# cc-ai/climategan

Measured on AMD Instinct MI355X. Metric: 640x640 images/sec (G+D step): per-domain sample slots per second of the joint Masker+Painter training step (update_G + update_D), global batch 32 per domain, higher is better.
Workload: dtype bf16

## Files before the change

### climategan_amd/csrc/conv1x1_xres.hip

```cpp
#include "conv_gemm.h"
#include <type_traits>

namespace {

typedef float f32x2 __attribute__((ext_vector_type(2)));

__device__ __attribute__((aligned(16))) unsigned int g_xres_zeros[4];

__device__ __forceinline__ float row16_sum_x(float v) {
  v += __builtin_bit_cast(float, __builtin_amdgcn_update_dpp(0, __builtin_bit_cast(int, v), 0x128, 0xf, 0xf, false));
  v += __builtin_bit_cast(float, __builtin_amdgcn_update_dpp(0, __builtin_bit_cast(int, v), 0x124, 0xf, 0xf, false));
  v += __builtin_bit_cast(float, __builtin_amdgcn_update_dpp(0, __builtin_bit_cast(int, v), 0x122, 0xf, 0xf, false));
  v += __builtin_bit_cast(float, __builtin_amdgcn_update_dpp(0, __builtin_bit_cast(int, v), 0x121, 0xf, 0xf, false));
  return v;
}

template <int I, int N, typename F>
__device__ __forceinline__ void static_for(F&& f) {
  if constexpr (I < N) {
    f(std::integral_constant<int, I>{});
    static_for<I + 1, N>(f);
  }
}

template <typename T, int KC, int PF>
__global__ __launch_bounds__(512, 1) void conv1x1_xres_kernel(ConvGemmArgs p, int npb, unsigned long long* ts) {
  constexpr int WC = 4, WP = 8;
  constexpr int NKS = 2 * KC;
  constexpr int XCHUNK = 32 * 1024;
  constexpr int ROWB = WC * 32 + 16;
  constexpr int STG = 16 * ROWB;
  static_assert(NKS % PF == 0, "the prefetch ring must divide the k-steps (static register indices)");
  static_assert(KC * XCHUNK + 8 * STG <= 160 * 1024, "LDS");
  extern __shared__ __attribute__((aligned(1024))) unsigned char smem[];

  const int lane = threadIdx.x & 63;
  const int wave = __builtin_amdgcn_readfirstlane(threadIdx.x >> 6);
  const int xcd = blockIdx.x & 7, slot = blockIdx.x >> 3;
  const int pblk = xcd * ((npb + 7) >> 3) + slot;
  if (pblk >= npb) return;
  auto stamp = [&](int i) {
    if (ts && lane == 0 && i < 16) ts[((size_t)blockIdx.x * 8 + wave) * 16 + i] = __builtin_readcyclecounter();
  };
  stamp(0);

  {
    const long zero_off = reinterpret_cast<const unsigned char*>(g_xres_zeros) - reinterpret_cast<const unsigned char*>(p.x);
    const int q = lane >> 3;
#pragma unroll
    for (int m = 0; m < KC * 4; ++m) {
      const int id = wave + 8 * m;
      const int cc2 = id >> 5, t = (id & 31) >> 1, half = id & 1;
      const int kchunk = (lane & 7) ^ (4 * half + ((q >> 1) & 3));
      const int pix = (pblk * 16 + t) * 16 + 8 * half + q;
      const long off = pix < p.npix ? ((long)pix * p.cin_s + cc2 * 64 + kchunk * 8) * 2 : zero_off;
      __builtin_amdgcn_global_load_lds(
          (const __attribute__((address_space(1))) void*)(reinterpret_cast<const unsigned char*>(p.x) + off),
          (__attribute__((address_space(3))) void*)(smem + id * 1024), 16, 0, 0);
    }
  }

  const int wc = wave & 3, wp = wave >> 2;
  const int j16 = lane & 15, g = lane >> 4;
  const int ncb = (p.ctiles + 15) >> 4;
  int b_off[2];
  {
    const int q = j16 & 7, h = j16 >> 3;
#pragma unroll
    for (int c = 0; c < 2; ++c) b_off[c] = wp * WP * 2048 + 1024 * h + 128 * q + 16 * ((4 * c + g) ^ (4 * h + ((q >> 1) & 3)));
  }
  const __amdgpu_buffer_rsrc_t rs_w =
      __builtin_amdgcn_make_buffer_rsrc(const_cast<u32x4*>(p.w), 0, p.ctiles * p.ksteps * 1024, 0x00020000);
  const __amdgpu_buffer_rsrc_t rs_y = __builtin_amdgcn_make_buffer_rsrc(p.y, 0, p.npix * p.cout_s * 2, 0x00020000);
  const int lane16 = lane * 16;
  u32x4 a[PF][WC];
  auto load_a = [&](auto slot_tag, int cb, int ks) {
    constexpr int sl = decltype(slot_tag)::value;
#pragma unroll
    for (int c = 0; c < WC; ++c) {
      const int ct = min(cb * 16 + wc * WC + c, p.ctiles - 1);
      a[sl][c] = __builtin_amdgcn_raw_buffer_load_b128(rs_w, lane16, (ct * p.ksteps + ks) * 1024, 0);
    }
  };
  static_for<0, PF>([&](auto i) { load_a(i, 0, decltype(i)::value); });

  asm volatile("s_waitcnt vmcnt(0)" ::: "memory");
  __builtin_amdgcn_s_barrier();
  stamp(1);

  unsigned char* stg = smem + KC * XCHUNK + wave * STG;
  const int st_rd = (lane >> 3) * ROWB + (lane & 7) * 16;
  const int st_voff = ((lane >> 3) * p.cout_s + (lane & 7) * 8) * 2;
  const int pix_wave = (pblk * 16 + wp * WP) * 16;

  u32x4 b_lo[4], b_hi[4];
  auto read_b = [&](u32x4* bh, int ks, int half) {
#pragma unroll
    for (int t = 0; t < 4; ++t)
      bh[t] = *reinterpret_cast<const u32x4*>(smem + (ks >> 1) * XCHUNK + b_off[ks & 1] + (half * 4 + t) * 2048);
  };

  for (int cb = 0; cb < ncb; ++cb) {
    read_b(b_lo, 0, 0);
    f32x4 acc[WC][WP];
#pragma unroll
    for (int c = 0; c < WC; ++c)
#pragma unroll
      for (int t = 0; t < WP; ++t) acc[c][t] = (f32x4){0.f, 0.f, 0.f, 0.f};

    auto kstep = [&](auto ks_tag) {
      constexpr int ks = decltype(ks_tag)::value;
      constexpr int sl = ks % PF;
      read_b(b_hi, ks, 1);
      __builtin_amdgcn_sched_barrier(0);
#pragma unroll
      for (int t = 0; t < 4; ++t)
#pragma unroll
        for (int c = 0; c < WC; ++c) acc[c][t] = mfma16(as_vec8<T>(a[sl][c]), as_vec8<T>(b_lo[t]), acc[c][t]);
      __builtin_amdgcn_sched_barrier(0);
      if constexpr (ks + 1 < NKS) read_b(b_lo, ks + 1, 0);
      __builtin_amdgcn_sched_barrier(0);
#pragma unroll
      for (int t = 0; t < 4; ++t)
#pragma unroll
        for (int c = 0; c < WC; ++c) acc[c][4 + t] = mfma16(as_vec8<T>(a[sl][c]), as_vec8<T>(b_hi[t]), acc[c][4 + t]);
      __builtin_amdgcn_sched_barrier(0);
      if constexpr (ks + PF < NKS) load_a(std::integral_constant<int, sl>{}, cb, ks + PF);
      __builtin_amdgcn_sched_barrier(0);
    };
    static_for<0, NKS>(kstep);
    stamp(2 + 2 * cb);

    const int cout_base = (cb * 16 + wc * WC) * 16;
    const bool full = pix_wave + WP * 16 <= p.npix && cout_base + WC * 16 <= p.cout_s;
    if (p.stats && pix_wave < p.npix) {
      const int chunk = pblk * 2 + wp;
      constexpr float inv_cnt = 1.f / (float)(WP * 16);
#pragma unroll
      for (int c = 0; c < WC; ++c) {
        f32x2 vr[WP][2];
#pragma unroll
        for (int t = 0; t < WP; ++t) {
#pragma unroll
          for (int hh = 0; hh < 2; ++hh) {
            float r0, r1;
            unpack2<T>(pack2<T>(acc[c][t][2 * hh], acc[c][t][2 * hh + 1]), r0, r1);
            vr[t][hh] = (f32x2){r0, r1};
          }
        }
        f32x2 s0[2] = {vr[0][0], vr[0][1]};
#pragma unroll
        for (int t = 1; t < WP; ++t) {
          s0[0] += vr[t][0];
          s0[1] += vr[t][1];
        }
        float mean[4];
#pragma unroll
        for (int r = 0; r < 4; ++r) mean[r] = row16_sum_x(s0[r >> 1][r & 1]) * inv_cnt;
        const f32x2 m2[2] = {(f32x2){mean[0], mean[1]}, (f32x2){mean[2], mean[3]}};
        f32x2 s1[2];
#pragma unroll
        for (int hh = 0; hh < 2; ++hh) {
          const f32x2 dv = vr[0][hh] - m2[hh];
          s1[hh] = dv * dv;
        }
#pragma unroll
        for (int t = 1; t < WP; ++t)
#pragma unroll
          for (int hh = 0; hh < 2; ++hh) {
            const f32x2 dv = vr[t][hh] - m2[hh];
            s1[hh] += dv * dv;
          }
        float o[8];
#pragma unroll
        for (int r = 0; r < 4; ++r) {
          o[2 * r] = mean[r];
          o[2 * r + 1] = row16_sum_x(s1[r >> 1][r & 1]);
        }
        const int ch = cout_base + c * 16 + 4 * g;
        if (j16 == 0 && ch < p.cout_s) {
          float* dst = p.stats + ((size_t)chunk * p.cout_s + ch) * 2;
          *reinterpret_cast<f32x4*>(dst) = (f32x4){o[0], o[1], o[2], o[3]};
          *reinterpret_cast<f32x4*>(dst + 4) = (f32x4){o[4], o[5], o[6], o[7]};
        }
      }
    }
    auto emit = [&](auto full_tag) {
      constexpr bool FULL = decltype(full_tag)::value;
#pragma unroll
      for (int t = 0; t < WP; ++t) {
#pragma unroll
        for (int c = 0; c < WC; ++c) {
          const f32x4 v = acc[c][t];
          *reinterpret_cast<u32x2*>(stg + j16 * ROWB + c * 32 + g * 8) = (u32x2){pack2<T>(v[0], v[1]), pack2<T>(v[2], v[3])};
        }
        asm volatile("s_waitcnt lgkmcnt(0)" ::: "memory");
#pragma unroll
        for (int it = 0; it < 2; ++it) {
          const u32x4 o = *reinterpret_cast<const u32x4*>(stg + st_rd + it * 8 * ROWB);
          const int pix0 = pix_wave + t * 16 + it * 8;
          if (FULL || (pix0 + (lane >> 3) < p.npix && cout_base + (lane & 7) * 8 < p.cout_s))
            __builtin_amdgcn_raw_buffer_store_b128(o, rs_y, st_voff, (pix0 * p.cout_s + cout_base) * 2, 2);
        }
        asm volatile("s_waitcnt lgkmcnt(0)" ::: "memory");
        if (t == WP / 2 - 1 && cb + 1 < ncb) {
          __builtin_amdgcn_sched_barrier(0);
          static_for<0, PF>([&](auto i) { load_a(i, cb + 1, decltype(i)::value); });
          __builtin_amdgcn_sched_barrier(0);
        }
      }
    };
    if (full) emit(std::true_type{});
    else emit(std::false_type{});
    stamp(3 + 2 * cb);
  }
}

CGAN_KNOB(unsigned long long*, g_xres_ts, nullptr);

template <typename T, int KC, int PF>
int launch_xres(const ConvGemmArgs& a, hipStream_t s) {
  constexpr size_t smem = (size_t)KC * 32 * 1024 + 8 * 16 * (4 * 32 + 16);
  static bool attr_set = false;
  if (!attr_set) {
    hipError_t e = hipFuncSetAttribute(reinterpret_cast<const void*>(&conv1x1_xres_kernel<T, KC, PF>),
                                       hipFuncAttributeMaxDynamicSharedMemorySize, 160 * 1024);
    if (e != hipSuccess) {
      cgan_set_error("conv1x1_xres: hipFuncSetAttribute failed: %s", hipGetErrorString(e));
      return CGAN_ERR_HIP;
    }
    attr_set = true;
  }
  const int npb = ceil_div(a.npix, 256);
  hipLaunchKernelGGL((conv1x1_xres_kernel<T, KC, PF>), dim3(ceil_div(npb, 8) * 8), dim3(512), smem, s, a, npb, g_xres_ts);
  return CGAN_OK;
}

template <typename T>
int launch_any(const ConvGemmArgs& a, hipStream_t s) {
  switch (a.cin_s >> 6) {
    case 1: return launch_xres<T, 1, 2>(a, s);
    case 2: return launch_xres<T, 2, 2>(a, s);
    case 3: return launch_xres<T, 3, 2>(a, s);
    default: return launch_xres<T, 4, 2>(a, s);
  }
}

}

CGAN_DEV_ONLY(extern "C" void cgan_debug_set_xres_tsbuf(void* p) { g_xres_ts = (unsigned long long*)p; })

bool conv1x1_xres_ok(const ConvGemmArgs& a) {
  return a.kh == 1 && a.kw == 1 && a.stride == 1 && a.pad == 0 && (a.cin_s & 63) == 0 && a.cin_s <= 256 && !a.has_res &&
         !a.bias && a.act == CGAN_ACT_NONE && a.cout == a.cout_s &&
         a.h_in == a.h_out && a.w_in == a.w_out && (long)a.npix * a.cin_s < (1L << 30) &&
         (long)a.npix * a.cout_s < (1L << 30);
}

int conv1x1_xres_launch(const ConvGemmArgs& a, int dtype, hipStream_t s) {
  return dtype == CGAN_F16 ? launch_any<F16>(a, s) : launch_any<BF16>(a, s);
}
```

### climategan_amd/csrc/conv_gemm.h

```cpp
#pragma once
#include "cgan_common.h"

struct ConvGemmArgs {
  const uint16_t* x;
  const u32x4* w;
  const float* bias;
  const uint16_t* res;
  const uint16_t* res2;
  uint16_t* y;
  int n, h_in, w_in, cin_s;
  int cout, cout_s, ctiles, ksteps;
  int kh, kw, stride, pad, dil, pad_mode;
  int h_out, w_out, npix;
  int act, has_res, res_ups;
  float slope;
  float* stats;
};

struct ConvGemmCls {
  int koff;
  int kh, kw;
  int offy, offx;
};
struct ConvGemmExtArgs {
  ConvGemmArgs a;
  int cls_s;
  int ksplit;
  int ks_per;
  float* ws;
  int pair;
  ConvGemmCls cls[4];
};
bool conv_gemm_ext_shape_ok(const ConvGemmArgs& a);
int conv_gemm_splitk_plan(const ConvGemmArgs& a);
size_t conv_gemm_splitk_workspace_bytes(const ConvGemmArgs& a, int ksplit);
int conv_gemm_splitk_launch(const ConvGemmArgs& a, int ksplit, float* ws, int dtype, hipStream_t s);
int conv_gemm_cls_launch(const ConvGemmArgs& a, int cls_s, const ConvGemmCls* cls, int dtype, hipStream_t s);
int conv_gemm_pair_launch(const ConvGemmArgs& a, int dtype, hipStream_t s);

bool conv_gemm_applicable(const CganConvDesc* d);
int conv_gemm_launch(const ConvGemmArgs& a, int dtype, hipStream_t s);
bool conv_gemm_res2_ok(const ConvGemmArgs& a, int dtype);
int conv_gemm_stats_chunk_pixels(const ConvGemmArgs& a, int dtype);
bool conv_gemm_big_ok(const ConvGemmArgs& a);
bool conv1x1_allc_ok(const ConvGemmArgs& a);
int conv1x1_allc_launch(const ConvGemmArgs& a, int dtype, hipStream_t s);
int conv_gemm_big_launch(const ConvGemmArgs& a, int dtype, hipStream_t s);
bool conv_gemm_big_pair_ok(const ConvGemmArgs& a, int dtype);
int conv_gemm_big_pair_launch(const ConvGemmArgs& a, int dtype, hipStream_t s);
bool conv1x1_xres_ok(const ConvGemmArgs& a);
int conv1x1_xres_launch(const ConvGemmArgs& a, int dtype, hipStream_t s);

#ifdef __HIPCC__
typedef float f32x2 __attribute__((ext_vector_type(2)));

__device__ __forceinline__ float row16_sum(float v) {
  v += __builtin_bit_cast(float, __builtin_amdgcn_update_dpp(0, __builtin_bit_cast(int, v), 0x128, 0xf, 0xf, false));
  v += __builtin_bit_cast(float, __builtin_amdgcn_update_dpp(0, __builtin_bit_cast(int, v), 0x124, 0xf, 0xf, false));
  v += __builtin_bit_cast(float, __builtin_amdgcn_update_dpp(0, __builtin_bit_cast(int, v), 0x122, 0xf, 0xf, false));
  v += __builtin_bit_cast(float, __builtin_amdgcn_update_dpp(0, __builtin_bit_cast(int, v), 0x121, 0xf, 0xf, false));
  return v;
}

template <typename T, int WC, int WP>
__device__ __forceinline__ void conv_gemm_stats_epilogue(f32x4 (&acc)[WC][WP], const ConvGemmArgs& p, int cout_base,
                                                         int chunk, int j, int g) {
  if (p.bias) {
#pragma unroll
    for (int c = 0; c < WC; ++c) {
      const int chb = cout_base + c * 16 + 4 * g;
      const f32x4 b = chb < p.cout_s ? *reinterpret_cast<const f32x4*>(p.bias + chb) : (f32x4){0.f, 0.f, 0.f, 0.f};
#pragma unroll
      for (int t = 0; t < WP; ++t) acc[c][t] += b;
    }
  }
  constexpr float inv_cnt = 1.f / (float)(WP * 16);
#pragma unroll
  for (int c = 0; c < WC; ++c) {
    f32x2 vr[WP][2];
#pragma unroll
    for (int t = 0; t < WP; ++t) {
#pragma unroll
      for (int hh = 0; hh < 2; ++hh) {
        float r0, r1;
        unpack2<T>(pack2<T>(acc[c][t][2 * hh], acc[c][t][2 * hh + 1]), r0, r1);
        vr[t][hh] = (f32x2){r0, r1};
      }
    }
    f32x2 s0[2] = {vr[0][0], vr[0][1]};
#pragma unroll
    for (int t = 1; t < WP; ++t) {
      s0[0] += vr[t][0];
      s0[1] += vr[t][1];
    }
    float sm[4], sq[4];
#pragma unroll
    for (int r = 0; r < 4; ++r) sm[r] = row16_sum(s0[r >> 1][r & 1]) * inv_cnt;
    const f32x2 m2[2] = {(f32x2){sm[0], sm[1]}, (f32x2){sm[2], sm[3]}};
    f32x2 s1[2];
#pragma unroll
    for (int hh = 0; hh < 2; ++hh) {
      const f32x2 dv = vr[0][hh] - m2[hh];
      s1[hh] = dv * dv;
    }
#pragma unroll
    for (int t = 1; t < WP; ++t)
#pragma unroll
      for (int hh = 0; hh < 2; ++hh) {
        const f32x2 dv = vr[t][hh] - m2[hh];
        s1[hh] += dv * dv;
      }
#pragma unroll
    for (int r = 0; r < 4; ++r) sq[r] = row16_sum(s1[r >> 1][r & 1]);
    const int ch = cout_base + c * 16 + 4 * g;
    if (j == 0 && ch < p.cout_s) {
      float o[8];
#pragma unroll
      for (int r = 0; r < 4; ++r) {
        o[2 * r] = sm[r];
        o[2 * r + 1] = sq[r];
      }
      float* dst = p.stats + ((size_t)chunk * p.cout_s + ch) * 2;
      *reinterpret_cast<f32x4*>(dst) = (f32x4){o[0], o[1], o[2], o[3]};
      *reinterpret_cast<f32x4*>(dst + 4) = (f32x4){o[4], o[5], o[6], o[7]};
    }
  }
}

template <typename T, int WC, int WP, int PP, bool RES2 = false>
__device__ __forceinline__ void conv_gemm_staged_store(const f32x4 (&acc)[WC][WP], const ConvGemmArgs& p,
                                                       unsigned char* stg, int pix0, int cout_base, const float* bias_ep,
                                                       int lane, int j, int g) {
  constexpr int ROWB = WC * 64 + 16;
  constexpr int CH = WC * 2;
  constexpr int NIT = PP * 16 * CH / 64;
  constexpr int NPASS = WP / PP;
  constexpr int PSTEP = 64 / CH;
  static_assert(64 % CH == 0 && WP % PP == 0, "a lane keeps its channel chunk over the iterations");
  const int qc = lane % CH, pl0 = lane / CH;
  const int ch = cout_base + qc * 8;
  const bool ch_ok = ch < p.cout_s;
  const bool plain = !bias_ep && !p.has_res && p.act == CGAN_ACT_NONE && p.cout == p.cout_s;
  f32x4 bb0 = (f32x4){0.f, 0.f, 0.f, 0.f}, bb1 = bb0;
  if (bias_ep && ch_ok) {
    bb0 = *reinterpret_cast<const f32x4*>(bias_ep + ch);
    bb1 = *reinterpret_cast<const f32x4*>(bias_ep + ch + 4);
  }
  u32x4 rv[NPASS][NIT];
  u32x4 rm[RES2 ? (NPASS > 1 ? 2 : 1) : 1][RES2 ? NIT : 1];
  auto load_rm = [&](int pass, u32x4 (&dst)[RES2 ? NIT : 1]) {
#pragma unroll
    for (int it = 0; it < (RES2 ? NIT : 0); ++it) {
      const int pix = pix0 + pass * PP * 16 + it * PSTEP + pl0;
      dst[it] = (u32x4){0u, 0u, 0u, 0u};
      if (pix < p.npix && ch_ok) dst[it] = CGAN_LD_STREAM(reinterpret_cast<const u32x4*>(p.res2 + (size_t)pix * p.cout_s + ch));
    }
  };
  if (p.has_res) {
#pragma unroll
    for (int pass = 0; pass < NPASS; ++pass)
#pragma unroll
      for (int it = 0; it < NIT; ++it) {
        const int pix = pix0 + pass * PP * 16 + it * PSTEP + pl0;
        rv[pass][it] = (u32x4){0u, 0u, 0u, 0u};
        if (pix < p.npix && ch_ok) {
          size_t rbase;
          if (p.res_ups) {
            const int ox = pix % p.w_out;
            const int r = pix / p.w_out;
            const int oy = r % p.h_out;
            const int nn = r / p.h_out;
            rbase = (((size_t)nn * (p.h_out >> 1) + (oy >> 1)) * (p.w_out >> 1) + (ox >> 1)) * p.cout_s;
          } else {
            rbase = (size_t)pix * p.cout_s;
          }
          rv[pass][it] = CGAN_LD_STREAM(reinterpret_cast<const u32x4*>(p.res + rbase + ch));
        }
      }
    if (RES2 && p.has_res == 3) load_rm(0, rm[0]);
    __builtin_amdgcn_sched_barrier(0);
  }
#pragma unroll
  for (int pass = 0; pass < NPASS; ++pass) {
#pragma unroll
    for (int tt = 0; tt < PP; ++tt)
#pragma unroll
      for (int c = 0; c < WC; ++c)
        *reinterpret_cast<f32x4*>(stg + (tt * 16 + j) * ROWB + c * 64 + g * 16) = acc[c][pass * PP + tt];
    asm volatile("s_waitcnt lgkmcnt(0)" ::: "memory");
    if (RES2 && NPASS > 1 && p.has_res == 3 && pass + 1 < NPASS) {
      __builtin_amdgcn_sched_barrier(0);
      load_rm(pass + 1, rm[(pass + 1) & 1]);
      __builtin_amdgcn_sched_barrier(0);
    }
    if (pass == 0 || (RES2 && p.has_res == 3 && pass >= 2)) __builtin_amdgcn_s_waitcnt(0x0F70);
#pragma unroll
    for (int it = 0; it < NIT; ++it) {
      const int pl = it * PSTEP + pl0;
      const int pix = pix0 + pass * PP * 16 + pl;
      const f32x4 v0 = *reinterpret_cast<const f32x4*>(stg + pl * ROWB + qc * 32);
      const f32x4 v1 = *reinterpret_cast<const f32x4*>(stg + pl * ROWB + qc * 32 + 16);
      float v[8] = {v0[0], v0[1], v0[2], v0[3], v1[0], v1[1], v1[2], v1[3]};
      if (!plain) {
        if (bias_ep) {
#pragma unroll
          for (int r = 0; r < 4; ++r) {
            v[r] += bb0[r];
            v[4 + r] += bb1[r];
          }
        }
        if (RES2 && p.has_res == 3) {
#pragma unroll
          for (int e = 0; e < 4; ++e) {
            float r0, r1, m0, m1;
            unpack2<T>(rv[pass][it][e], r0, r1);
            unpack2<T>(rm[RES2 && NPASS > 1 ? (pass & 1) : 0][RES2 ? it : 0][e], m0, m1);
            v[2 * e] = cgan_res_apply3(v[2 * e], r0, m0);
            v[2 * e + 1] = cgan_res_apply3(v[2 * e + 1], r1, m1);
          }
        } else if (p.has_res) {
#pragma unroll
          for (int e = 0; e < 4; ++e) {
            float r0, r1;
            unpack2<T>(rv[pass][it][e], r0, r1);
            v[2 * e] = cgan_res_apply(v[2 * e], r0, p.has_res);
            v[2 * e + 1] = cgan_res_apply(v[2 * e + 1], r1, p.has_res);
          }
        }
        act_apply_n(v, p.act, p.slope);
        if (p.cout < p.cout_s) {
#pragma unroll
          for (int r = 0; r < 8; ++r)
            if (ch + r >= p.cout) v[r] = 0.f;
        }
      }
      u32x4 o;
#pragma unroll
      for (int e = 0; e < 4; ++e) o[e] = pack2<T>(v[2 * e], v[2 * e + 1]);
      if (pix < p.npix && ch_ok) CGAN_ST_STREAM(o, reinterpret_cast<u32x4*>(p.y + (size_t)pix * p.cout_s + ch));
    }
    asm volatile("s_waitcnt lgkmcnt(0)" ::: "memory");
  }
}
#endif
```

### climategan_amd/csrc/conv_gemm.hip

```cpp
#include "conv_gemm.h"
#include <type_traits>

namespace {

__device__ __attribute__((aligned(16))) unsigned int g_gemm_zeros[4];

constexpr int NSTAGE = 3;
CGAN_KNOB(int, g_gemm_ws, 0);

__device__ __forceinline__ int reflect_i(int i, int n) {
  if (i < 0) i = -i;
  if (i >= n) i = 2 * n - 2 - i;
  return i;
}

template <typename T, int WAVES_C, int WC, int WP, bool REFLECT, int NS = NSTAGE, bool RES2 = false>
__global__ __launch_bounds__(256, 2) void conv_gemm_kernel(ConvGemmArgs p, int npb, int ncb) {
  constexpr int WAVES_P = 4 / WAVES_C;
  constexpr int CT_BLK = WAVES_C * WC;
  constexpr int PT_BLK = WAVES_P * WP;
  constexpr int STAGE_BYTES = (CT_BLK + PT_BLK) * 1024;
  constexpr int W_PER_WAVE = CT_BLK / 4;
  constexpr int P_PER_WAVE = PT_BLK / 4;
  constexpr int DMA_PER_WAVE = W_PER_WAVE + P_PER_WAVE;
// ... 124 lines not shown
  conv_gemm_staged_store<T, WC, WP, PP, RES2>(acc, p, stg, (pblk * PT_BLK + wp * WP) * 16, cout_base, bias_ep, lane, j, g);
}

template <typename T, int WC, int WP>
__global__ __launch_bounds__(512, 2) void conv_gemm_k64_kernel(ConvGemmArgs p, int npb, int ncb, int tiles_total) {
  constexpr int CT_BLK = 2 * WC, PT_BLK = 2 * WP;
  constexpr int W_BYTES = CT_BLK * 2048, STAGE_BYTES = (CT_BLK + PT_BLK) * 2048;
  constexpr int NS = 3;
  constexpr int W_PER = CT_BLK / 2, P_PER = PT_BLK / 2, PIECES = W_PER + P_PER;
  static_assert(PIECES <= 63, "vmcnt range");
  extern __shared__ __attribute__((aligned(1024))) unsigned char smem[];

  const int lane = threadIdx.x & 63;
  const int wave = __builtin_amdgcn_readfirstlane(threadIdx.x >> 6);
  const int xcd = blockIdx.x & 7, slot = blockIdx.x >> 3, nslot = gridDim.x >> 3;
  const int per = (tiles_total + 7) >> 3;
  const int t0 = xcd * per;
  const int t1 = min(t0 + per, tiles_total);
  const int my_n = (t1 - t0 > slot) ? (t1 - t0 - slot + nslot - 1) / nslot : 0;
  if (my_n <= 0) return;
  const int first = t0 + slot;
  const int cc2n = p.cin_s >> 6;
  const int n_st = p.kh * p.kw * cc2n;
  const int n_it = my_n * n_st;

  if (wave >= 4) {
    const int pw = wave - 4;
    const int half = pw & 1;
    const int ccn = p.cin_s >> 5;
    const long zero_off = reinterpret_cast<const unsigned char*>(g_gemm_zeros) - reinterpret_cast<const unsigned char*>(p.x);
    const int q = lane >> 3;
    const int kchunk = (lane & 7) ^ (4 * half + ((q >> 1) & 3));
    int poff[P_PER];
    unsigned vmask[P_PER];
    const u32x4* wtile[W_PER];
    auto set_tile = [&](int ti) {
      const int gt = first + ti * nslot;
      const int pblk = gt / ncb;
      const int cblk = gt - pblk * ncb;
#pragma unroll
      for (int m = 0; m < W_PER; ++m)
        wtile[m] = p.w + (size_t)min(cblk * CT_BLK + (pw >> 1) + 2 * m, p.ctiles - 1) * p.ksteps * 64 + half * 64 + lane;
#pragma unroll
      for (int m = 0; m < P_PER; ++m) {
        const int pix = (pblk * PT_BLK + (pw >> 1) + 2 * m) * 16 + 8 * half + q;
        const bool v = pix < p.npix;
        const int pc = v ? pix : 0;
        const int ox = pc % p.w_out;
        const int r = pc / p.w_out;
        const int oy = r % p.h_out;
        const int nn = r / p.h_out;
        const int py0 = oy * p.stride - p.pad, px0 = ox * p.stride - p.pad;
        poff[m] = ((nn * p.h_in * p.w_in + py0 * p.w_in + px0) * p.cin_s + kchunk * 8) * 2;
        unsigned mk = 0;
        for (int ky = 0; ky < p.kh; ++ky)
          for (int kx = 0; kx < p.kw; ++kx) {
            const bool ok = v && (unsigned)(py0 + ky * p.dil) < (unsigned)p.h_in && (unsigned)(px0 + kx * p.dil) < (unsigned)p.w_in;
            mk |= (ok ? 1u : 0u) << (ky * p.kw + kx);
          }
        vmask[m] = mk;
      }
    };
    int i_ky = 0, i_kx = 0, i_cc2 = 0, i_buf = 0, i_st = 0, i_tile = 0, issued = 0;
    auto issue_stage = [&]() {
      unsigned char* buf = smem + i_buf * STAGE_BYTES;
      const int tap = i_ky * p.kw + i_kx;
      const size_t w_ks = (size_t)(tap * ccn + 2 * i_cc2) * 64;
#pragma unroll
      for (int m = 0; m < W_PER; ++m)
        __builtin_amdgcn_global_load_lds((const __attribute__((address_space(1))) void*)(wtile[m] + w_ks),
                                         (__attribute__((address_space(3))) void*)(buf + (pw + 4 * m) * 1024), 16, 0, 0);
      const int tap_off = ((i_ky * p.w_in + i_kx) * p.dil * p.cin_s + i_cc2 * 64) * 2;
#pragma unroll
      for (int m = 0; m < P_PER; ++m) {
        const long off = ((vmask[m] >> tap) & 1u) ? (long)(poff[m] + tap_off) : zero_off;
        const unsigned char* src = reinterpret_cast<const unsigned char*>(p.x) + off;
        __builtin_amdgcn_global_load_lds((const __attribute__((address_space(1))) void*)src,
                                         (__attribute__((address_space(3))) void*)(buf + W_BYTES + (pw + 4 * m) * 1024), 16, 0, 0);
      }
      ++issued;
      i_buf = (i_buf + 1 == NS) ? 0 : i_buf + 1;
      if (++i_st == n_st) {
        i_st = 0; i_ky = 0; i_kx = 0; i_cc2 = 0;
        if (++i_tile < my_n) set_tile(i_tile);
      } else if (++i_kx == p.kw) {
        i_kx = 0;
        if (++i_ky == p.kh) {
          i_ky = 0;
          ++i_cc2;
        }
      }
    };
    set_tile(0);
    for (int s2 = 0; s2 < NS - 1; ++s2)
      if (issued < n_it) issue_stage();
    for (int j = 0; j < n_it; ++j) {
      if (issued - 1 - j >= NS - 2)
        asm volatile("s_waitcnt vmcnt(%0)" ::"n"((NS - 2) * PIECES) : "memory");
      else
        asm volatile("s_waitcnt vmcnt(0)" ::: "memory");
      __builtin_amdgcn_s_barrier();
      if (issued < n_it) issue_stage();
    }
    return;
  }

  const int wc = wave & 1, wp = wave >> 1;
  const int j16 = lane & 15, g = lane >> 4;
  f32x4 acc[WC][WP];
#pragma unroll
  for (int c = 0; c < WC; ++c)
#pragma unroll
    for (int t = 0; t < WP; ++t) acc[c][t] = (f32x4){0.f, 0.f, 0.f, 0.f};
  u32x4 a0[WC], b0[WP], a1[WC], b1[WP];
  int r_buf = 0;
  const int a_off = wc * WC * 2048 + lane * 16;
  int b_off[2];
  {
    const int q = j16 & 7, h = j16 >> 3;
#pragma unroll
    for (int c = 0; c < 2; ++c)
      b_off[c] = W_BYTES + wp * WP * 2048 + 1024 * h + 128 * q + 16 * ((4 * c + g) ^ (4 * h + ((q >> 1) & 3)));
  }
  auto fetch_one = [&](const unsigned char* buf, int c, int qi, u32x4* na, u32x4* nb) {
    if (qi < WP)
      nb[qi] = *reinterpret_cast<const u32x4*>(buf + b_off[c] + qi * 2048);
    else
      na[qi - WP] = *reinterpret_cast<const u32x4*>(buf + a_off + ((qi - WP) * 2 + c) * 1024);
  };
  auto step = [&](const u32x4* ca, const u32x4* cb, u32x4* na, u32x4* nb, int next_half) {
    __builtin_amdgcn_sched_barrier(0);
    if (next_half == 0) {
      asm volatile("s_waitcnt lgkmcnt(0)" ::: "memory");
      __builtin_amdgcn_s_barrier();
      r_buf = (r_buf + 1 == NS) ? 0 : r_buf + 1;
    }
    __builtin_amdgcn_sched_barrier(0);
    const unsigned char* buf = smem + r_buf * STAGE_BYTES;
    constexpr int NM = WC * WP, NR = WC + WP;
    constexpr int EVERY = NM / NR >= 2 ? 2 : 1;
#pragma unroll
    for (int i = 0; i < NM; ++i) {
      const int c = i / WP, t = i % WP;
      acc[c][t] = mfma16(as_vec8<T>(ca[c]), as_vec8<T>(cb[t]), acc[c][t]);
      if (next_half >= 0 && i % EVERY == EVERY - 1 && i / EVERY < NR) {
        fetch_one(buf, next_half, i / EVERY, na, nb);
        __builtin_amdgcn_sched_barrier(0);
      }
    }
    __builtin_amdgcn_sched_barrier(0);
  };
  auto first_read = [&](bool advance) {
    asm volatile("s_waitcnt lgkmcnt(0)" ::: "memory");
    __builtin_amdgcn_s_barrier();
    if (advance) r_buf = (r_buf + 1 == NS) ? 0 : r_buf + 1;
    const unsigned char* buf = smem + r_buf * STAGE_BYTES;
#pragma unroll
    for (int qi = 0; qi < WC + WP; ++qi) fetch_one(buf, 0, qi, a0, b0);
  };
  auto epilogue = [&](int ti) {
    const int gt = first + ti * nslot;
    const int pblk = gt / ncb;
    const int cblk = gt - pblk * ncb;
    uint2 rv[WP][WC];
    if (p.has_res) {
#pragma unroll
      for (int t = 0; t < WP; ++t) {
        const int pix = (pblk * PT_BLK + wp * WP + t) * 16 + j16;
        size_t rbase = 0;
        if (pix < p.npix) {
          if (p.res_ups) {
            int ox = pix % p.w_out;
            int r = pix / p.w_out;
            int oy = r % p.h_out;
            int nn = r / p.h_out;
            rbase = (((size_t)nn * (p.h_out >> 1) + (oy >> 1)) * (p.w_out >> 1) + (ox >> 1)) * p.cout_s;
          } else {
            rbase = (size_t)pix * p.cout_s;
          }
        }
#pragma unroll
        for (int c = 0; c < WC; ++c) {
          const int ch = (cblk * CT_BLK + wc * WC + c) * 16 + 4 * g;
          rv[t][c] = make_uint2(0u, 0u);
          if (pix < p.npix && ch < p.cout_s) rv[t][c] = *reinterpret_cast<const uint2*>(p.res + rbase + ch);
        }
      }
      __builtin_amdgcn_sched_barrier(0);
      __builtin_amdgcn_s_waitcnt(0x0F70);
    }
#pragma unroll
    for (int t = 0; t < WP; ++t) {
      const int pix = (pblk * PT_BLK + wp * WP + t) * 16 + j16;
#pragma unroll
      for (int c = 0; c < WC; ++c) {
        const int ch = (cblk * CT_BLK + wc * WC + c) * 16 + 4 * g;
        float v[4] = {acc[c][t][0], acc[c][t][1], acc[c][t][2], acc[c][t][3]};
        acc[c][t] = (f32x4){0.f, 0.f, 0.f, 0.f};
        if (pix >= p.npix || ch >= p.cout_s) continue;
        if (p.bias) {
#pragma unroll
          for (int r = 0; r < 4; ++r) v[r] += p.bias[ch + r];
        }
        if (p.has_res) {
          float r0, r1;
          unpack2<T>(rv[t][c].x, r0, r1);
          v[0] = cgan_res_apply(v[0], r0, p.has_res); v[1] = cgan_res_apply(v[1], r1, p.has_res);
          unpack2<T>(rv[t][c].y, r0, r1);
          v[2] = cgan_res_apply(v[2], r0, p.has_res); v[3] = cgan_res_apply(v[3], r1, p.has_res);
        }
#pragma unroll
        for (int r = 0; r < 4; ++r) {
          v[r] = act_apply(v[r], p.act, p.slope);
          if (ch + r >= p.cout) v[r] = 0.f;
        }
        u32x2 o;
        o.x = pack2<T>(v[0], v[1]);
        o.y = pack2<T>(v[2], v[3]);
        CGAN_ST_STREAM(o, reinterpret_cast<u32x2*>(p.y + (size_t)pix * p.cout_s + ch));
      }
    }
  };

  for (int ti = 0; ti < my_n; ++ti) {
    first_read(ti > 0);
    for (int st = 0; st + 1 < n_st; ++st) {
      step(a0, b0, a1, b1, 1);
      step(a1, b1, a0, b0, 0);
    }
    step(a0, b0, a1, b1, 1);
    step(a1, b1, a0, b0, -1);
    epilogue(ti);
  }
}

template <typename T, int WC, int WP>
int launch_k64(const ConvGemmArgs& a, hipStream_t s) {
  constexpr int CT_BLK = 2 * WC, PT_BLK = 2 * WP;
  constexpr size_t smem = (size_t)3 * (CT_BLK + PT_BLK) * 2048;
  static bool attr_set = false;
  if (!attr_set) {
    hipError_t e = hipFuncSetAttribute(reinterpret_cast<const void*>(&conv_gemm_k64_kernel<T, WC, WP>),
                                       hipFuncAttributeMaxDynamicSharedMemorySize, 160 * 1024);
    if (e != hipSuccess) {
      cgan_set_error("conv_gemm_k64: hipFuncSetAttribute failed: %s", hipGetErrorString(e));
      return CGAN_ERR_HIP;
    }
    attr_set = true;
  }
  const int npb = ceil_div(ceil_div(a.npix, 16), PT_BLK);
  const int ncb = ceil_div(a.ctiles, CT_BLK);
  const int tiles = npb * ncb;
  const int per = ceil_div(tiles, 8);
  const int nslot = per < 32 ? per : 32;
  hipLaunchKernelGGL((conv_gemm_k64_kernel<T, WC, WP>), dim3(8 * nslot), dim3(512), smem, s, a, npb, ncb, tiles);
  return CGAN_OK;
}
bool k64_ok(const ConvGemmArgs& a) {
  return (a.cin_s & 63) == 0 && a.pad_mode != CGAN_PAD_REFLECT && a.kh * a.kw <= 32 &&
         (long)a.n * a.h_in * a.w_in * a.cin_s < (1L << 30) - (1L << 20);
}


template <typename T, int WAVES_C, int WC, int WP, bool REFLECT, int NS = NSTAGE, bool RES2 = false>
int launch_cfg2(const ConvGemmArgs& a, hipStream_t s) {
  constexpr int WAVES_P = 4 / WAVES_C;
  constexpr int CT_BLK = WAVES_C * WC, PT_BLK = WAVES_P * WP;
  constexpr size_t smem = (size_t)NS * (CT_BLK + PT_BLK) * 1024;
  static bool attr_set = false;
  if (!attr_set) {
    hipError_t e = hipFuncSetAttribute(reinterpret_cast<const void*>(&conv_gemm_kernel<T, WAVES_C, WC, WP, REFLECT, NS, RES2>),
                                       hipFuncAttributeMaxDynamicSharedMemorySize, 160 * 1024);
    if (e != hipSuccess) {
      cgan_set_error("conv_gemm: hipFuncSetAttribute failed: %s", hipGetErrorString(e));
      return CGAN_ERR_HIP;
    }
    attr_set = true;
  }
  const int npb = ceil_div(ceil_div(a.npix, 16), PT_BLK);
  const int ncb = ceil_div(a.ctiles, CT_BLK);
  const int grid = ceil_div(npb, 8) * 8 * ncb;
  hipLaunchKernelGGL((conv_gemm_kernel<T, WAVES_C, WC, WP, REFLECT, NS, RES2>), dim3(grid), dim3(256), smem, s, a, npb, ncb);
  return CGAN_OK;
}

template <typename T, int WAVES_C, int WC, int WP, int NS = NSTAGE>
int launch_cfg(const ConvGemmArgs& a, hipStream_t s) {
  return a.pad_mode == CGAN_PAD_REFLECT ? launch_cfg2<T, WAVES_C, WC, WP, true, NS>(a, s)
                                        : launch_cfg2<T, WAVES_C, WC, WP, false, NS>(a, s);
}

CGAN_KNOB(int, g_gemm_cfg, 0);

enum { KIND_PLAIN = 0, KIND_K64_256x128, KIND_K64_128x256, KIND_BIG, KIND_DIRECT, KIND_XRES };
struct Choice {
  int kind;
  int cfg;
};

Choice choose(const ConvGemmArgs& a, bool bf16) {
  const int ptiles = ceil_div(a.npix, 16);
  const bool no_big = g_gemm_ws == 9;
  const bool no_xres = g_gemm_ws == 9 || g_gemm_ws == 12;
  const int ws = (no_big || no_xres || g_gemm_ws == 13 || g_gemm_ws == 14) ? 0 : g_gemm_ws;
  switch (ws) {
    case 5: if (k64_ok(a)) return {KIND_K64_256x128, 0}; break;
    case 6: if (k64_ok(a)) return {KIND_K64_128x256, 0}; break;
    case 8: if (conv_gemm_big_ok(a)) return {KIND_BIG, 0}; break;
    case 10: if (conv1x1_allc_ok(a)) return {KIND_DIRECT, 0}; break;
    case 11: if (conv1x1_xres_ok(a)) return {KIND_XRES, 0}; break;
    default: break;
  }
  const bool automatic = ws == 0 && g_gemm_cfg == 0;
  (void)bf16;
  if (automatic && !no_big && conv1x1_allc_ok(a) && a.ctiles <= 4 && a.npix >= 16384) return {KIND_DIRECT, 0};
  if (automatic && !no_xres && conv1x1_xres_ok(a) && a.ctiles >= 16 && a.npix >= 16384) return {KIND_XRES, 0};
  const bool long_1x1 = a.kh * a.kw == 1 && g_gemm_ws != 13 &&
                        (g_gemm_ws == 14 ? (a.cin_s >= 2048 || (a.cin_s >= 512 && a.ctiles >= 128))
                                         : (a.cin_s >= 1024 || (a.cin_s >= 512 && a.ctiles >= 128)));
  if (automatic && !no_big && conv_gemm_big_ok(a) && a.npix >= 16384 &&
      ((a.cin_s * a.kh * a.kw >= 4096 && a.cin_s >= 512 && !(a.kh * a.kw >= 9 && a.cin_s >= 2048)) || long_1x1))
    return {KIND_BIG, 0};
  if (automatic && k64_ok(a) && a.kh * a.kw >= 9 && a.cin_s >= 512 && a.npix >= 16384) return {KIND_K64_256x128, 0};
  switch (g_gemm_cfg) {
    case 1: return {KIND_PLAIN, 1};
    case 2: if (a.ctiles <= 16) return {KIND_PLAIN, 2}; break;
    case 3: return {KIND_PLAIN, 3};
    case 4: return {KIND_PLAIN, 4};
    case 5: return {KIND_PLAIN, 5};
    default: break;
  }
  if (a.ctiles <= 4) return {KIND_PLAIN, 1};
  if (a.kh * a.kw == 1 && a.ksteps <= 16) return {KIND_PLAIN, 5};
  if (a.ctiles > 8 && a.ctiles <= 16 && ceil_div(ptiles, 8) >= 384) return {KIND_PLAIN, 2};
  if ((long)ceil_div(ptiles, 16) * ceil_div(a.ctiles, 8) >= 384) return {KIND_PLAIN, 3};
  return {KIND_PLAIN, 4};
}

template <typename T>
int launch(const ConvGemmArgs& a, hipStream_t s) {
  const Choice ch = choose(a, std::is_same<T, BF16>::value);
  switch (ch.kind) {
    case KIND_K64_256x128: return launch_k64<T, 8, 4>(a, s);
    case KIND_K64_128x256: return launch_k64<T, 4, 8>(a, s);
    case KIND_BIG: return conv_gemm_big_launch(a, T::id, s);
    case KIND_DIRECT: return conv1x1_allc_launch(a, T::id, s);
    case KIND_XRES: return conv1x1_xres_launch(a, T::id, s);
    default: break;
  }
  switch (ch.cfg) {
    case 1: return launch_cfg<T, 1, 4, 4>(a, s);
    case 2: return launch_cfg<T, 2, 8, 4>(a, s);
    case 3: return launch_cfg<T, 2, 4, 8>(a, s);
    case 5:
      if (a.has_res == 3) return launch_cfg2<T, 2, 4, 4, false, 2, true>(a, s);
      return launch_cfg<T, 2, 4, 4, 2>(a, s);
    default: return launch_cfg<T, 2, 4, 4>(a, s);
  }
}

}

bool conv_gemm_applicable(const CganConvDesc* d) {
  const int cin_s = cgan_cs(d->c_in), cout_s = cgan_cs(d->c_out);
  const long npix = (long)d->n * d->h_out * d->w_out;
  const long in_elems = (long)d->n * d->h_in * d->w_in * cin_s;
  return (cin_s % 32) == 0 && cout_s >= 64 && !d->in_upsample && npix >= 2048 && in_elems < (1L << 31) - (1L << 20) &&
         (long)ceil_div((int)ceil_div((int)npix, 16), 8) * ceil_div(ceil_div(cout_s, 16), 8) >= 128;
}

CGAN_DEV_ONLY(extern "C" void cgan_debug_set_gemm_cfg(int v) { g_gemm_cfg = v; })
CGAN_DEV_ONLY(extern "C" void cgan_debug_set_gemm_ws(int v) { g_gemm_ws = v; })

int conv_gemm_launch(const ConvGemmArgs& a, int dtype, hipStream_t s) {
  return dtype == CGAN_F16 ? launch<F16>(a, s) : launch<BF16>(a, s);
}

bool conv_gemm_res2_ok(const ConvGemmArgs& a, int dtype) {
  const Choice ch = choose(a, dtype == CGAN_BF16);
  return (ch.kind == KIND_PLAIN && ch.cfg == 5 && a.pad_mode != CGAN_PAD_REFLECT) || ch.kind == KIND_BIG;
}

int conv_gemm_stats_chunk_pixels(const ConvGemmArgs& a, int dtype) {
  const Choice ch = choose(a, dtype == CGAN_BF16);
  if (ch.kind == KIND_XRES) return a.npix % 128 == 0 ? 128 : 0;
  if (ch.kind == KIND_BIG) return a.npix % 64 == 0 ? 64 : 0;
  if (ch.kind != KIND_PLAIN) return 0;
  const int ppb = ch.cfg == 3 ? 128 : 64;
  return a.npix % ppb == 0 ? ppb : 0;
}
```

Baseline: 55.63.

## Add persistent streaming variant of xres 1x1 conv with double-buffered input tiles

Adds a STREAM mode to the resident-input 1x1 conv kernel. The grid is capped at the CU count and each block loops over pixel tiles. Input tiles are double-buffered in LDS and prefetched by one wave group while the other computes, and all 8 waves are spread across output channels (32 ctiles per block) instead of 2x4. It is selected automatically when ctiles >= 32. The aim is to remove per-block fill latency and launch tail by overlapping the next tile's DMA with the MFMA and epilogue, at the cost of more complex synchronization with hand-written m0/vmcnt asm and halved pixel tile size.

```diff
diff --git a/climategan_amd/csrc/conv1x1_xres.hip b/climategan_amd/csrc/conv1x1_xres.hip
--- a/climategan_amd/csrc/conv1x1_xres.hip
+++ b/climategan_amd/csrc/conv1x1_xres.hip
@@ -1,4 +1,5 @@
 #include "conv_gemm.h"
+#include <algorithm>
 #include <type_traits>
 
 namespace {
@@ -23,46 +24,70 @@
   }
 }
 
-template <typename T, int KC, int PF>
+__device__ __forceinline__ void xres_dma16(const unsigned char* sbase, unsigned voff, const unsigned char* lds_dst) {
+  const unsigned lds = (unsigned)reinterpret_cast<size_t>((__attribute__((address_space(3))) const unsigned char*)lds_dst);
+  unsigned keep;
+  asm volatile("s_mov_b32 %0, m0\n\ts_mov_b32 m0, %2\n\ts_nop 0\n\tglobal_load_lds_dwordx4 %1, %3\n\ts_mov_b32 m0, %0"
+               : "=&s"(keep)
+               : "v"(voff), "s"(lds), "s"(sbase)
+               : "memory");
+}
+
+template <typename T, int KC, int PF, bool STREAM>
 __global__ __launch_bounds__(512, 1) void conv1x1_xres_kernel(ConvGemmArgs p, int npb, unsigned long long* ts) {
   constexpr int WC = 4, WP = 8;
+  constexpr int WAVES_P = STREAM ? 1 : 2, WAVES_C = 8 / WAVES_P;
+  constexpr int CB_TILES = WAVES_C * WC;
+  constexpr int TPT = WAVES_P * WP;
   constexpr int NKS = 2 * KC;
-  constexpr int XCHUNK = 32 * 1024;
+  constexpr int XCHUNK = TPT * 2048;
+  constexpr int XBUF = KC * XCHUNK;
+  constexpr int NPIECE = XBUF / 8192;
   constexpr int ROWB = WC * 32 + 16;
   constexpr int STG = 16 * ROWB;
   static_assert(NKS % PF == 0, "the prefetch ring must divide the k-steps (static register indices)");
-  static_assert(KC * XCHUNK + 8 * STG <= 160 * 1024, "LDS");
+  static_assert((STREAM ? 2 : 1) * XBUF + 8 * STG <= 160 * 1024, "LDS");
   extern __shared__ __attribute__((aligned(1024))) unsigned char smem[];
 
   const int lane = threadIdx.x & 63;
   const int wave = __builtin_amdgcn_readfirstlane(threadIdx.x >> 6);
   const int xcd = blockIdx.x & 7, slot = blockIdx.x >> 3;
-  const int pblk = xcd * ((npb + 7) >> 3) + slot;
+  const int pblk = xcd * (STREAM ? (int)(gridDim.x >> 3) : ((npb + 7) >> 3)) + slot;
   if (pblk >= npb) return;
+  const int ntl = STREAM ? (npb - pblk + (int)gridDim.x - 1) / (int)gridDim.x : 1;
   auto stamp = [&](int i) {
-    if (ts && lane == 0 && i < 16) ts[((size_t)blockIdx.x * 8 + wave) * 16 + i] = __builtin_readcyclecounter();
+    if (ts && lane == 0 && i < (STREAM ? 14 : 16)) ts[((size_t)blockIdx.x * 8 + wave) * 16 + i] = __builtin_readcyclecounter();
   };
   stamp(0);
 
-  {
-    const long zero_off = reinterpret_cast<const unsigned char*>(g_xres_zeros) - reinterpret_cast<const unsigned char*>(p.x);
+  const long zero_off = reinterpret_cast<const unsigned char*>(g_xres_zeros) - reinterpret_cast<const unsigned char*>(p.x);
+  auto fill = [&](int tile, int buf) {
+    if constexpr (STREAM) asm volatile("" : "+s"(tile));
     const int q = lane >> 3;
 #pragma unroll
-    for (int m = 0; m < KC * 4; ++m) {
+    for (int m = 0; m < NPIECE; ++m) {
       const int id = wave + 8 * m;
-      const int cc2 = id >> 5, t = (id & 31) >> 1, half = id & 1;
+      const int cc2 = id / (2 * TPT), t = (id % (2 * TPT)) >> 1, half = id & 1;
       const int kchunk = (lane & 7) ^ (4 * half + ((q >> 1) & 3));
-      const int pix = (pblk * 16 + t) * 16 + 8 * half + q;
-      const long off = pix < p.npix ? ((long)pix * p.cin_s + cc2 * 64 + kchunk * 8) * 2 : zero_off;
-      __builtin_amdgcn_global_load_lds(
-          (const __attribute__((address_space(1))) void*)(reinterpret_cast<const unsigned char*>(p.x) + off),
-          (__attribute__((address_space(3))) void*)(smem + id * 1024), 16, 0, 0);
-    }
-  }
-
-  const int wc = wave & 3, wp = wave >> 2;
+      const int pix = (tile * TPT + t) * 16 + 8 * half + q;
+      if constexpr (STREAM) {
+        const unsigned voff = (unsigned)(min(pix, p.npix - 1) * p.cin_s + kchunk * 8) * 2u;
+        xres_dma16(reinterpret_cast<const unsigned char*>(p.x) + cc2 * 128, voff, smem + buf * XBUF + id * 1024);
+      } else {
+        const long off = pix < p.npix ? ((long)pix * p.cin_s + cc2 * 64 + kchunk * 8) * 2 : zero_off;
+        __builtin_amdgcn_global_load_lds(
+            (const __attribute__((address_space(1))) void*)(reinterpret_cast<const unsigned char*>(p.x) + off),
+            (__attribute__((address_space(3))) void*)(smem + id * 1024), 16, 0, 0);
+      }
+    }
+  };
+  fill(pblk, 0);
+
+  const int wc = STREAM ? wave : (wave & 3), wp = STREAM ? 0 : (wave >> 2);
+  const int grp = wave >> 2;
+  const int gstep = STREAM ? (int)gridDim.x : 0;
   const int j16 = lane & 15, g = lane >> 4;
-  const int ncb = (p.ctiles + 15) >> 4;
+  const int ncb = (p.ctiles + CB_TILES - 1) / CB_TILES;
   int b_off[2];
   {
     const int q = j16 & 7, h = j16 >> 3;
@@ -78,7 +103,7 @@
     constexpr int sl = decltype(slot_tag)::value;
 #pragma unroll
     for (int c = 0; c < WC; ++c) {
-      const int ct = min(cb * 16 + wc * WC + c, p.ctiles - 1);
+      const int ct = min(cb * CB_TILES + wc * WC + c, p.ctiles - 1);
       a[sl][c] = __builtin_amdgcn_raw_buffer_load_b128(rs_w, lane16, (ct * p.ksteps + ks) * 1024, 0);
     }
   };
@@ -87,21 +112,31 @@
   asm volatile("s_waitcnt vmcnt(0)" ::: "memory");
   __builtin_amdgcn_s_barrier();
   stamp(1);
-
-  unsigned char* stg = smem + KC * XCHUNK + wave * STG;
+  if (STREAM && grp == 1 && ntl > 1) fill(pblk + gstep, 1);
+
+  unsigned char* stg = smem + (STREAM ? 2 : 1) * XBUF + wave * STG;
   const int st_rd = (lane >> 3) * ROWB + (lane & 7) * 16;
   const int st_voff = ((lane >> 3) * p.cout_s + (lane & 7) * 8) * 2;
-  const int pix_wave = (pblk * 16 + wp * WP) * 16;
 
   u32x4 b_lo[4], b_hi[4];
-  auto read_b = [&](u32x4* bh, int ks, int half) {
+  auto read_b = [&](u32x4* bh, int xb, int ks, int half) {
 #pragma unroll
     for (int t = 0; t < 4; ++t)
-      bh[t] = *reinterpret_cast<const u32x4*>(smem + (ks >> 1) * XCHUNK + b_off[ks & 1] + (half * 4 + t) * 2048);
+      bh[t] = *reinterpret_cast<const u32x4*>(smem + xb + (ks >> 1) * XCHUNK + b_off[ks & 1] + (half * 4 + t) * 2048);
   };
 
+  bool drained = false;
+  for (int i = 0; i < ntl; ++i) {
+  const int tile = pblk + i * gstep;
+  const int xb = (i & 1) * XBUF;
+  const int pix_wave = (tile * TPT + wp * WP) * 16;
+  if (STREAM && grp == 0 && i > 0) {
+    if (drained) asm volatile("s_waitcnt vmcnt(16)" ::: "memory");
+    else asm volatile("s_waitcnt vmcnt(0)" ::: "memory");
+    __builtin_amdgcn_s_barrier();
+  }
   for (int cb = 0; cb < ncb; ++cb) {
-    read_b(b_lo, 0, 0);
+    read_b(b_lo, xb, 0, 0);
     f32x4 acc[WC][WP];
 #pragma unroll
     for (int c = 0; c < WC; ++c)
@@ -111,14 +146,14 @@
     auto kstep = [&](auto ks_tag) {
       constexpr int ks = decltype(ks_tag)::value;
       constexpr int sl = ks % PF;
-      read_b(b_hi, ks, 1);
+      read_b(b_hi, xb, ks, 1);
       __builtin_amdgcn_sched_barrier(0);
 #pragma unroll
       for (int t = 0; t < 4; ++t)
 #pragma unroll
         for (int c = 0; c < WC; ++c) acc[c][t] = mfma16(as_vec8<T>(a[sl][c]), as_vec8<T>(b_lo[t]), acc[c][t]);
       __builtin_amdgcn_sched_barrier(0);
-      if constexpr (ks + 1 < NKS) read_b(b_lo, ks + 1, 0);
+      if constexpr (ks + 1 < NKS) read_b(b_lo, xb, ks + 1, 0);
       __builtin_amdgcn_sched_barrier(0);
 #pragma unroll
       for (int t = 0; t < 4; ++t)
@@ -129,12 +164,22 @@
       __builtin_amdgcn_sched_barrier(0);
     };
     static_for<0, NKS>(kstep);
-    stamp(2 + 2 * cb);
-
-    const int cout_base = (cb * 16 + wc * WC) * 16;
+    stamp(2 + 2 * (i * ncb + cb));
+    if (STREAM && i + 1 < ntl) {
+      if (grp == 1 && cb == ncb - 1) {
+        asm volatile("s_waitcnt vmcnt(0)" ::: "memory");
+        __builtin_amdgcn_s_barrier();
+        if (i + 2 < ntl) fill(tile + 2 * gstep, i & 1);
+      }
+      if (grp == 0 && cb == 0) fill(tile + gstep, (i + 1) & 1);
+    }
+    const bool more = cb + 1 < ncb || i + 1 < ntl;
+    const int cb_next = cb + 1 < ncb ? cb + 1 : 0;
+
+    const int cout_base = (cb * CB_TILES + wc * WC) * 16;
     const bool full = pix_wave + WP * 16 <= p.npix && cout_base + WC * 16 <= p.cout_s;
     if (p.stats && pix_wave < p.npix) {
-      const int chunk = pblk * 2 + wp;
+      const int chunk = tile * WAVES_P + wp;
       constexpr float inv_cnt = 1.f / (float)(WP * 16);
 #pragma unroll
       for (int c = 0; c < WC; ++c) {
@@ -185,10 +230,11 @@
         }
       }
     }
-    auto emit = [&](auto full_tag) {
+    auto emit = [&](auto full_tag, auto half_tag) {
       constexpr bool FULL = decltype(full_tag)::value;
-#pragma unroll
-      for (int t = 0; t < WP; ++t) {
+      constexpr int T0 = decltype(half_tag)::value * (WP / 2);
+#pragma unroll
+      for (int t = T0; t < T0 + WP / 2; ++t) {
 #pragma unroll
         for (int c = 0; c < WC; ++c) {
           const f32x4 v = acc[c][t];
@@ -203,46 +249,82 @@
             __builtin_amdgcn_raw_buffer_store_b128(o, rs_y, st_voff, (pix0 * p.cout_s + cout_base) * 2, 2);
         }
         asm volatile("s_waitcnt lgkmcnt(0)" ::: "memory");
-        if (t == WP / 2 - 1 && cb + 1 < ncb) {
-          __builtin_amdgcn_sched_barrier(0);
-          static_for<0, PF>([&](auto i) { load_a(i, cb + 1, decltype(i)::value); });
-          __builtin_amdgcn_sched_barrier(0);
-        }
       }
     };
-    if (full) emit(std::true_type{});
-    else emit(std::false_type{});
-    stamp(3 + 2 * cb);
+    using H0 = std::integral_constant<int, 0>;
+    using H1 = std::integral_constant<int, 1>;
+    auto prefetch = [&]() {
+      if (STREAM || more) {
+        __builtin_amdgcn_sched_barrier(0);
+        static_for<0, PF>([&](auto k) { load_a(k, cb_next, decltype(k)::value); });
+        __builtin_amdgcn_sched_barrier(0);
+      }
+    };
+    if constexpr (STREAM) {
+      if (full) emit(std::true_type{}, H0{});
+      else emit(std::false_type{}, H0{});
+      prefetch();
+      if (full) emit(std::true_type{}, H1{});
+      else emit(std::false_type{}, H1{});
+    } else if (full) {
+      emit(std::true_type{}, H0{});
+      prefetch();
+      emit(std::true_type{}, H1{});
+    } else {
+      emit(std::false_type{}, H0{});
+      prefetch();
+      emit(std::false_type{}, H1{});
+    }
+    drained = full;
+    stamp(3 + 2 * (i * ncb + cb));
+  }
+  }
+  if (STREAM && ts && lane == 0) {
+    ts[((size_t)blockIdx.x * 8 + wave) * 16 + 14] = __builtin_amdgcn_s_getreg(4 | (31 << 11));
+    ts[((size_t)blockIdx.x * 8 + wave) * 16 + 15] = __builtin_readcyclecounter();
   }
 }
 
 CGAN_KNOB(unsigned long long*, g_xres_ts, nullptr);
 
-template <typename T, int KC, int PF>
+template <typename T, int KC, int PF, bool STREAM>
 int launch_xres(const ConvGemmArgs& a, hipStream_t s) {
-  constexpr size_t smem = (size_t)KC * 32 * 1024 + 8 * 16 * (4 * 32 + 16);
+  constexpr size_t smem = (size_t)KC * (STREAM ? 2 * 16 : 32) * 1024 + 8 * 16 * (4 * 32 + 16);
   static bool attr_set = false;
+  static int ncu = 0;
   if (!attr_set) {
-    hipError_t e = hipFuncSetAttribute(reinterpret_cast<const void*>(&conv1x1_xres_kernel<T, KC, PF>),
+    hipError_t e = hipFuncSetAttribute(reinterpret_cast<const void*>(&conv1x1_xres_kernel<T, KC, PF, STREAM>),
                                        hipFuncAttributeMaxDynamicSharedMemorySize, 160 * 1024);
     if (e != hipSuccess) {
       cgan_set_error("conv1x1_xres: hipFuncSetAttribute failed: %s", hipGetErrorString(e));
       return CGAN_ERR_HIP;
     }
+    int dev = 0;
+    if (hipGetDevice(&dev) != hipSuccess || hipDeviceGetAttribute(&ncu, hipDeviceAttributeMultiprocessorCount, dev) != hipSuccess ||
+        ncu < 8) {
+      cgan_set_error("conv1x1_xres: cannot read the device's compute-unit count");
+      return CGAN_ERR_HIP;
+    }
     attr_set = true;
   }
+  if (STREAM) {
+    const int ntile = ceil_div(a.npix, 128);
+    const int grid = std::min(ceil_div(ntile, 8) * 8, ncu / 8 * 8);
+    hipLaunchKernelGGL((conv1x1_xres_kernel<T, KC, PF, true>), dim3(grid), dim3(512), smem, s, a, ntile, g_xres_ts);
+    return CGAN_OK;
+  }
   const int npb = ceil_div(a.npix, 256);
-  hipLaunchKernelGGL((conv1x1_xres_kernel<T, KC, PF>), dim3(ceil_div(npb, 8) * 8), dim3(512), smem, s, a, npb, g_xres_ts);
+  hipLaunchKernelGGL((conv1x1_xres_kernel<T, KC, PF, STREAM>), dim3(ceil_div(npb, 8) * 8), dim3(512), smem, s, a, npb, g_xres_ts);
   return CGAN_OK;
 }
 
-template <typename T>
+template <typename T, bool STREAM>
 int launch_any(const ConvGemmArgs& a, hipStream_t s) {
   switch (a.cin_s >> 6) {
-    case 1: return launch_xres<T, 1, 2>(a, s);
-    case 2: return launch_xres<T, 2, 2>(a, s);
-    case 3: return launch_xres<T, 3, 2>(a, s);
-    default: return launch_xres<T, 4, 2>(a, s);
+    case 1: return launch_xres<T, 1, 2, STREAM>(a, s);
+    case 2: return launch_xres<T, 2, 2, STREAM>(a, s);
+    case 3: return launch_xres<T, 3, 2, STREAM>(a, s);
+    default: return launch_xres<T, 4, 2, STREAM>(a, s);
   }
 }
 
@@ -257,6 +339,9 @@
          (long)a.npix * a.cout_s < (1L << 30);
 }
 
-int conv1x1_xres_launch(const ConvGemmArgs& a, int dtype, hipStream_t s) {
-  return dtype == CGAN_F16 ? launch_any<F16>(a, s) : launch_any<BF16>(a, s);
-}
+bool conv1x1_xres_stream_ok(const ConvGemmArgs& a) { return conv1x1_xres_ok(a) && a.ctiles >= 32; }
+
+int conv1x1_xres_launch(const ConvGemmArgs& a, int dtype, bool stream, hipStream_t s) {
+  if (stream) return dtype == CGAN_F16 ? launch_any<F16, true>(a, s) : launch_any<BF16, true>(a, s);
+  return dtype == CGAN_F16 ? launch_any<F16, false>(a, s) : launch_any<BF16, false>(a, s);
+}
diff --git a/climategan_amd/csrc/conv_gemm.h b/climategan_amd/csrc/conv_gemm.h
--- a/climategan_amd/csrc/conv_gemm.h
+++ b/climategan_amd/csrc/conv_gemm.h
@@ -49,7 +49,8 @@
 bool conv_gemm_big_pair_ok(const ConvGemmArgs& a, int dtype);
 int conv_gemm_big_pair_launch(const ConvGemmArgs& a, int dtype, hipStream_t s);
 bool conv1x1_xres_ok(const ConvGemmArgs& a);
-int conv1x1_xres_launch(const ConvGemmArgs& a, int dtype, hipStream_t s);
+bool conv1x1_xres_stream_ok(const ConvGemmArgs& a);
+int conv1x1_xres_launch(const ConvGemmArgs& a, int dtype, bool stream, hipStream_t s);
 
 #ifdef __HIPCC__
 typedef float f32x2 __attribute__((ext_vector_type(2)));
diff --git a/climategan_amd/csrc/conv_gemm.hip b/climategan_amd/csrc/conv_gemm.hip
--- a/climategan_amd/csrc/conv_gemm.hip
+++ b/climategan_amd/csrc/conv_gemm.hip
@@ -450,19 +450,22 @@
   const int ptiles = ceil_div(a.npix, 16);
   const bool no_big = g_gemm_ws == 9;
   const bool no_xres = g_gemm_ws == 9 || g_gemm_ws == 12;
-  const int ws = (no_big || no_xres || g_gemm_ws == 13 || g_gemm_ws == 14) ? 0 : g_gemm_ws;
+  const bool no_stream = g_gemm_ws == 15;
+  const int ws = (no_big || no_xres || no_stream || g_gemm_ws == 13 || g_gemm_ws == 14) ? 0 : g_gemm_ws;
   switch (ws) {
     case 5: if (k64_ok(a)) return {KIND_K64_256x128, 0}; break;
     case 6: if (k64_ok(a)) return {KIND_K64_128x256, 0}; break;
     case 8: if (conv_gemm_big_ok(a)) return {KIND_BIG, 0}; break;
     case 10: if (conv1x1_allc_ok(a)) return {KIND_DIRECT, 0}; break;
     case 11: if (conv1x1_xres_ok(a)) return {KIND_XRES, 0}; break;
+    case 16: if (conv1x1_xres_stream_ok(a)) return {KIND_XRES, 1}; break;
     default: break;
   }
   const bool automatic = ws == 0 && g_gemm_cfg == 0;
   (void)bf16;
   if (automatic && !no_big && conv1x1_allc_ok(a) && a.ctiles <= 4 && a.npix >= 16384) return {KIND_DIRECT, 0};
-  if (automatic && !no_xres && conv1x1_xres_ok(a) && a.ctiles >= 16 && a.npix >= 16384) return {KIND_XRES, 0};
+  if (automatic && !no_xres && conv1x1_xres_ok(a) && a.ctiles >= 16 && a.npix >= 16384)
+    return {KIND_XRES, !no_stream && conv1x1_xres_stream_ok(a) ? 1 : 0};
   const bool long_1x1 = a.kh * a.kw == 1 && g_gemm_ws != 13 &&
                         (g_gemm_ws == 14 ? (a.cin_s >= 2048 || (a.cin_s >= 512 && a.ctiles >= 128))
                                          : (a.cin_s >= 1024 || (a.cin_s >= 512 && a.ctiles >= 128)));
@@ -493,7 +496,7 @@
     case KIND_K64_128x256: return launch_k64<T, 4, 8>(a, s);
     case KIND_BIG: return conv_gemm_big_launch(a, T::id, s);
     case KIND_DIRECT: return conv1x1_allc_launch(a, T::id, s);
-    case KIND_XRES: return conv1x1_xres_launch(a, T::id, s);
+    case KIND_XRES: return conv1x1_xres_launch(a, T::id, ch.cfg == 1, s);
     default: break;
   }
   switch (ch.cfg) {
```

Result: no change. 55.75, median of 5 (+0.2%).
